# vpc-ccg/circminer

Measured on AMD Instinct MI355X. Metric: paired reads/sec (whole node), hg38 k=20, 2x150 bp; circ_report bit-exact, higher is better.
Workload: dtype int32/u8 (chain scores f64)

## Files before the change

circminer_amd/csrc/cm_core.h:

```cpp
#pragma once
#include <stdint.h>

#include "circminer_hot.h"
#if defined(CM_STAGE2_HOST)
#include <vector>
#endif

#if defined(__HIPCC__)
#define CM_HD __host__ __device__
#define CM_NOINLINE inline
#else
#define CM_HD
#define CM_NOINLINE
#endif

#if !defined(CM_HOOK_DP)
#define CM_HOOK_DP(kind, s, n, t, m) ((void)0)
#endif
#if defined(CM_STATS) && !defined(__HIPCC__)
#if !defined(CM_NSTATS)
#define CM_NSTATS 16
#endif
extern "C" unsigned long long cm_stats[CM_NSTATS];
#define CM_STAT(i, n) ((i) < CM_NSTATS ? (void)(cm_stats[(i) < CM_NSTATS ? (i) : 0] += (unsigned long long)(n)) : (void)0)
// ... 94 lines not shown
constexpr uint32_t MAXUB = 4294967295u;
constexpr int MAXDISCRDTLEN = 20000;
constexpr uint32_t LARIAT2BEGTH = 1000u;
constexpr int DPTINF = 10000000;
constexpr int SC_MAT = 1, SC_MIS = -3, SC_IND = -3, SC_XD = 8;
constexpr int MAX_SEEDS = CM_MAX_CHAIN_FRAGS;
constexpr int MAX_BAND = 8;
constexpr int MAX_TID = 64;
#if defined(CM_STAGE2_HOST)
constexpr int MEMO_N = 512;
#elif defined(CM_MEMO_N)
constexpr int MEMO_N = CM_MEMO_N;
#else
constexpr int MEMO_N = 8;
#endif

enum { ERR_POOL = 1, ERR_SEEDS = 4, ERR_BAND = 8, ERR_MEMO = 16 };

struct KCore {
    cm_params P;
    cm_index_view X;
    AnnotDev A;
    const uint32_t *desc = nullptr;
};
struct Core {
    cm_params P;
    IndexV X;
    AnnotV A;
    g_u32 desc = nullptr;
};
CM_HD inline Core to_core(const KCore &k) {
    Core c;
    c.P = k.P;
    c.X = to_dev(k.X);
    c.A = to_dev(k.A);
    c.desc = (g_u32)k.desc;
    return c;
}

template <class T> CM_HD inline T cmin(T a, T b) { return a < b ? a : b; }
template <class T> CM_HD inline T cmax(T a, T b) { return a > b ? a : b; }
CM_HD inline int cabs(int a) { return a < 0 ? -a : a; }

struct SV {
    g_u8 p;
    int32_t off;
    int32_t step;
    int32_t mode;
    CM_HD inline SV sub(int a) const { return SV{p, off + a * step, step, mode}; }
    CM_HD inline SV rev(int m) const { return SV{p, off + (m - 1) * step, -step, mode}; }
};
struct Read {
    g_u8 p;
    int32_t len;
    int32_t rc;
    CM_HD inline SV view() const { return rc ? SV{p, len - 1, -1, 1} : SV{p, 0, 1, 0}; }
};


// ... 209 lines not shown
        if (e12end < 0 || beg2s2 < 0) continue;
        trans_dist = e12end + beg2s2;
        if (cabs(trans_dist - read_dist) <= c.P.max_ed) return true;
    }
    if (td2intron != -1) {
        trans_dist = td2intron;
        return true;
    }
    trans_dist = INF_I;
    return false;
}

constexpr int SMALL_W = 32;
struct ChainStoreGlobal {
    ChainWork &w;
    g_u32 POS;
    const uint32_t *start;
    const uint32_t *cnt_;
    const uint32_t *base_;
    uint32_t lb_[MAX_SEEDS];
    CM_G Event *ev;
    uint32_t n_ev, cap_ev;
    bool lost;
    CM_HD ChainStoreGlobal(ChainWork &ww, g_u32 pos, const uint32_t *st, const uint32_t *cn, const uint32_t *bs)
        : w(ww), POS(pos), start(st), cnt_(cn), base_(bs), ev(nullptr), n_ev(0), cap_ev(0), lost(false) {}
    CM_HD inline uint32_t cnt(int s) const { return cnt_[s]; }
    CM_HD inline uint32_t base(int s) const { return base_[s]; }
    CM_HD inline uint32_t total(int kc) const { return base_[kc]; }
    CM_HD inline void lb_reset(int kc) { for (int k = 0; k < kc; ++k) lb_[k] = 0; }
    CM_HD inline uint32_t lb(int s) const { return lb_[s]; }
    CM_HD inline void set_lb(int s, uint32_t v) { lb_[s] = v; }
    CM_HD inline void init(uint32_t n_cells, double v) {
        for (uint32_t x = 0; x < n_cells; ++x) {
            w.dp_score[x] = v;
            w.dp_prev[x] = -1;
        }
    }
    CM_HD inline uint32_t pos(int s, uint32_t i) const { return POS[start[s] + i]; }
    CM_HD inline double score(uint32_t x) const { return w.dp_score[x]; }
    CM_HD inline int32_t prev(uint32_t x) const { return w.dp_prev[x]; }
    CM_HD inline void set(uint32_t x, double sc, int32_t pv) {
        w.dp_score[x] = sc;
        w.dp_prev[x] = pv;
    }
    CM_HD inline void push(double sc, uint32_t cell) {
        if (n_ev == cap_ev && !lost) {
            const uint32_t ncap = cap_ev ? cap_ev * 4u : 32u;
            const unsigned long long bytes = (unsigned long long)ncap * sizeof(Event);
            const unsigned long long off = pool_take(w.pool_cursor, bytes);
            if (off + bytes > w.pool_bytes) {
                lost = true;
                flag_err(w.err, ERR_POOL);
            } else {
                CM_G Event *ne = (CM_G Event *)(w.pool + off);
                for (uint32_t q = 0; q < n_ev; ++q) ne[q] = ev[q];
                ev = ne;
                cap_ev = ncap;
            }
        }
        if (n_ev < cap_ev) {
            ev[n_ev].score = sc;
            ev[n_ev].cell = cell;
            ++n_ev;
        }
    }
    CM_HD inline uint32_t n_events() const { return n_ev; }
// ... 1904 lines not shown
```

circminer_amd/csrc/cm_hot.hip:

```cpp
#include <chrono>
#include <hip/hip_runtime.h>
#include <rocprim/device/device_radix_sort.hpp>

#include <algorithm>
#include <atomic>
#include <cstdarg>
#include <cstdio>
#include <cstdlib>
#include <cstring>
#include <string>
#include <functional>
#include <thread>
#include <vector>

#include "circminer_hot.h"
#include "cm_core.h"
#include "cm_aos.h"
#include "cm_index_build.h"

using cmc::Core;
using cmc::KCore;

namespace {

// ... 289 lines not shown
                                                         const int32_t *nchain, const int32_t *high, cm_mapped_read *state, uint8_t *active, int32_t *cat,
                                                         int is_last, int *err, unsigned long long *counters, int str_cap,
                                                         unsigned long long *lane_clk, const uint32_t *perm, const unsigned int *n_light,
                                                         unsigned int *next_chunk, RetryArgs ra) {
    pair_kernel<false>(kc, rd, pair0, n_tile, chains, nchain, high, state, active, cat, is_last, err, counters, str_cap, lane_clk, perm, n_light, next_chunk, ra);
}

template <class T> __device__ inline T wave_excl_scan(T v, int lane, T &total) {
    T x = v;
    for (int o = 1; o < 64; o <<= 1) {
        const T y = __shfl_up(x, o);
        if (lane >= o) x += y;
    }
    total = __shfl(x, 63);
    return x - v;
}
struct HeavyChainCtx {
#if defined(CM_CHAIN_DIAG)
    unsigned long long *tk;
#endif
    const Core *c;
    CM_L const uint32_t *LP;
    CM_L const uint32_t *NB;
    const uint32_t *base, *cnt;
    int kc, seq_len;
    CM_G double *dps;
    CM_G int32_t *dpp;
};
__device__ inline uint32_t heavy_cell(const HeavyChainCtx &h, int ii, uint32_t i, CM_G cmc::Event *ev, double &out_score, int32_t &out_prev,
                                     double &e0, double &e1) {
    const Core &c = *h.c;
    const int kmer = c.P.kmer;
    const uint32_t read_remain = (uint32_t)(h.seq_len - ii * kmer - kmer);
    const int32_t cur_info = (int32_t)h.LP[h.base[ii] + i];
    const uint32_t seg_start = (uint32_t)cur_info, seg_end = (uint32_t)cur_info + kmer - 1;
    uint32_t max_lpos_lim = cmc::MAXUB, max_exon_end = 0;
    int ol = -1;
    double my_score = (double)kmer;
    int32_t my_prev = -1;
    uint32_t n = 0;
    const uint32_t cell = h.base[ii] + i;
    const bool near = (h.NB[cell >> 5] >> (cell & 31)) & 1u;
    uint2 parked = make_uint2(0u, 0u);
    int parked_ol = -1;
    if (near) {
        parked = *(CM_G const uint2 *)(h.dps + cell);
        parked_ol = h.dpp[cell];
    }
#if defined(CM_CHAIN_DIAG)
    if (!ev) h.tk[3] += 1;
#define CD_T0 const unsigned long long cd_t = wall_clock64()
#define CD_ADD(k) h.tk[k] += wall_clock64() - cd_t
#else
#define CD_T0
#define CD_ADD(k)
#endif
    for (int jj = ii + 1; jj < h.kc; ++jj) {
        const uint32_t pcn = h.cnt[jj];
        if (pcn == 0) continue;
        CM_L const uint32_t *pp = h.LP + h.base[jj];
        uint32_t lo = 0, hi = pcn;
        {
            CD_T0;
            while (lo < hi) {
                const uint32_t mid = (lo + hi) >> 1;
                if ((int32_t)pp[mid] <= cur_info) lo = mid + 1;
                else hi = mid;
            }
            CD_ADD(0);
        }
        if (lo >= pcn) continue;
        if (cur_info + c.P.max_intron < (int32_t)pp[lo]) continue;
        if (max_lpos_lim == cmc::MAXUB) {
            CD_T0;
            if (near) {
                max_lpos_lim = parked.x;
                max_exon_end = parked.y;
                ol = parked_ol;
            } else {
                max_exon_end = 0;
                ol = -1;
                max_lpos_lim = seg_start + read_remain + (uint32_t)c.P.max_ed;
            }
            CD_ADD(1);
        }
        const int distr = (jj - ii) * kmer - kmer;
        CD_T0;
        for (uint32_t j = lo; j < pcn && pp[j] <= max_lpos_lim; ++j) {
#if defined(CM_CHAIN_DIAG)
            if (!ev) h.tk[4] += 1;
#endif
            const uint32_t pinfo = pp[j];
            int genome_dist, distt, trans_dist;
            if (max_exon_end == 0 || (pinfo + kmer - 1) <= max_exon_end) genome_dist = (int)(pinfo - seg_end - 1);
            else genome_dist = cmc::INF_I;
            if (cmc::cabs(genome_dist - distr) <= c.P.max_ed) distt = genome_dist;
            else if (cmc::check_junction(c, seg_start, pinfo, ol, kmer, distr, trans_dist)) distt = trans_dist;
            else continue;
            const int maxd = distr < distt ? distt : distr, mind = distr < distt ? distr : distt;
            const double beta = 0.1 * (double)(maxd - mind);
            const double alpha = 2e4 * (double)kmer;
            const double t1 = h.dps[h.base[jj] + j] + alpha;
            const double temp_score = t1 - beta;
            if (temp_score > my_score) {
                my_score = temp_score;
                my_prev = (int32_t)(((uint32_t)jj << 16) | j);
                if (ev) {
                    ev[n].score = temp_score;
                    ev[n].cell = ((uint32_t)ii << 16) | i;
                }
                if (n == 0) e0 = temp_score;
                else if (n == 1) e1 = temp_score;
                ++n;
            }
        }
        CD_ADD(2);
    }
    out_score = my_score;
    out_prev = my_prev;
    return n;
}

struct HeavyBackTrack {
    uint32_t base[cmc::MAX_SEEDS + 1];
    uint32_t cand[CM_BESTCHAINLIM + 2];
// ... 21 lines not shown
    const uint32_t max_best = (uint32_t)c.P.max_chain_len;
    const unsigned int n_heavy = *n_perm;
    auto take = [&]() { return (unsigned int)__shfl((int)(lane == 0 ? atomicAdd(next_problem, 1u) : 0u), 0); };
    for (unsigned int hidx = take(); hidx < n_heavy; hidx = take()) {
        const uint32_t r = perm[hidx];
        const uint64_t p = pair0 + (r >> 2);
        const int mate = (int)((r >> 1) & 1u);
        const int len = (int)(mate ? rd.off2[p + 1] - rd.off2[p] : rd.off1[p + 1] - rd.off1[p]);
#if defined(CM_CHAIN_DIAG)
        const unsigned long long dg0 = wall_clock64();
#endif
        uint32_t st[cmc::MAX_SEEDS], cn[cmc::MAX_SEEDS], base[cmc::MAX_SEEDS + 1];
        int kc = S;
        for (int s = 0; s < S; ++s) {
            st[s] = sstart[(uint64_t)r * S + s];
            cn[s] = scnt[(uint64_t)r * S + s];
        }
        while (kc >= 1 && cn[kc - 1] == 0) --kc;
        base[0] = 0;
        for (int s = 0; s < kc; ++s) base[s + 1] = base[s] + cn[s];
        const uint32_t ncell = base[kc];
        CM_G double *dps = (CM_G double *)(dp_score + celloff[r]);
        CM_G int32_t *dpp = (CM_G int32_t *)(dp_prev + celloff[r]);
        for (int s = 0; s < kc; ++s)
            for (uint32_t i = lane; i < cn[s]; i += 64) LP[base[s] + i] = c.X.pos[st[s] + i];
        for (uint32_t x = lane; x < ncell; x += 64) {
            dps[x] = (double)kmer;
            dpp[x] = -1;
        }
        __threadfence_block();
        __syncthreads();
        CM_L uint32_t *NB = LP + ncell;
        CM_L uint16_t *Q = (CM_L uint16_t *)(NB + 2 * ((ncell + 63) >> 6));
        {
            const uint32_t n_pre = kc >= 1 ? base[kc - 1] : 0u;
            const unsigned long long lt = (1ull << lane) - 1ull;
            uint32_t qn = 0;
            auto look_up = [&](uint32_t cnt) {
                if ((uint32_t)lane < cnt) {
                    const uint32_t x = Q[lane];
                    int ii = 0;
                    for (int s = 1; s < kc; ++s) ii += x >= base[s] ? 1 : 0;
                    const uint32_t read_remain = (uint32_t)(len - ii * kmer - kmer);
                    uint32_t mx = 0;
                    int ol = -1;
                    const uint32_t lim = cmc::upper_bound_lookup(c, LP[x], (uint32_t)kmer, read_remain, mx, ol);
                    *(CM_G uint2 *)(dps + x) = make_uint2(lim, mx);
                    dpp[x] = ol;
                }
            };
            for (uint32_t x0 = 0; x0 < n_pre; x0 += 256) {
                bool nr[4];
#pragma unroll
                for (int u = 0; u < 4; ++u) {
                    const uint32_t x = x0 + 64 * u + lane;
                    nr[u] = x < n_pre && cmc::bit_at(c.A.near_border_bits, c.A.n_bits, LP[x]);
                }
#pragma unroll
                for (int u = 0; u < 4; ++u) {
                    const uint32_t xb = x0 + 64 * u;
                    if (xb >= n_pre) break;
                    const unsigned long long m = __ballot(nr[u]);
                    if (lane == 0) NB[xb >> 5] = (uint32_t)m;
                    if (lane == 32) NB[(xb >> 5) + 1] = (uint32_t)(m >> 32);
                    if (nr[u]) Q[qn + __popcll(m & lt)] = (uint16_t)(xb + lane);
                    qn += (uint32_t)__popcll(m);
                }
                __syncthreads();
                while (qn >= 64) {
                    look_up(64);
                    uint16_t keep[4];
#pragma unroll
                    for (int u = 0; u < 4; ++u) keep[u] = 64u * u + (uint32_t)lane < qn - 64 ? Q[64 + 64 * u + lane] : (uint16_t)0;
                    __syncthreads();
#pragma unroll
                    for (int u = 0; u < 4; ++u)
                        if (64u * u + (uint32_t)lane < qn - 64) Q[64 * u + lane] = keep[u];
                    qn -= 64;
                    __syncthreads();
                }
            }
            if (qn) look_up(qn);
        }
        __threadfence_block();
        __syncthreads();
#if defined(CM_CHAIN_DIAG)
        const unsigned long long dg1 = wall_clock64();
#endif
#if defined(CM_CHAIN_DIAG)
        unsigned long long tk[5] = {0, 0, 0, 0, 0};
        unsigned long long wv[4] = {0, 0, 0, 0};
        HeavyChainCtx H{tk, &c, LP, NB, base, cn, kc, len, dps, dpp};
#else
        HeavyChainCtx H{&c, LP, NB, base, cn, kc, len, dps, dpp};
#endif
        CM_G cmc::Event *ev = nullptr;
        uint32_t n_ev = 0, cap_ev = 0;
        bool lost = false;
        for (int ii = kc - 2; ii >= 0; --ii) {
            for (uint32_t i0 = 0; i0 < cn[ii]; i0 += 64) {
                const uint32_t i = i0 + lane;
                const bool on = i < cn[ii];
                double sc = 0, e0 = 0, e1 = 0;
                int32_t pv = -1;
#if defined(CM_CHAIN_DIAG)
                const unsigned long long w0 = wall_clock64();
#endif
                const uint32_t mine = on ? heavy_cell(H, ii, i, (CM_G cmc::Event *)nullptr, sc, pv, e0, e1) : 0u;
#if defined(CM_CHAIN_DIAG)
                const unsigned long long w1 = wall_clock64();
#endif
                uint32_t total;
                const uint32_t off = wave_excl_scan(mine, lane, total);
                if (n_ev + total > cap_ev && !lost) {
                    uint32_t ncap = cap_ev ? cap_ev : 256u;
                    while (ncap < n_ev + total) ncap *= 4u;
                    const unsigned long long bytes = (unsigned long long)ncap * sizeof(cmc::Event);
                    unsigned long long o = 0;
                    if (lane == 0) o = atomicAdd(pool_cursor, bytes);
                    o = ((unsigned long long)__shfl((unsigned int)(o >> 32), 0) << 32) | (unsigned long long)__shfl((unsigned int)o, 0);
                    if (o + bytes > pool_bytes) {
                        lost = true;
                        if (lane == 0) atomicOr(err, cmc::ERR_POOL);
                    } else {
                        CM_G cmc::Event *ne = (CM_G cmc::Event *)((CM_G uint8_t *)pool + o);
                        for (uint32_t q = lane; q < n_ev; q += 64) ne[q] = ev[q];
                        ev = ne;
                        cap_ev = ncap;
                    }
                }
                if (on) {
                    if (mine && !lost) {
                        CM_G cmc::Event *dst = ev + n_ev + off;
                        if (mine <= 2) {
                            dst[0].score = e0;
                            dst[0].cell = ((uint32_t)ii << 16) | i;
                            if (mine == 2) {
                                dst[1].score = e1;
                                dst[1].cell = ((uint32_t)ii << 16) | i;
                            }
                        } else heavy_cell(H, ii, i, dst, sc, pv, e0, e1);
                    }
                    dps[base[ii] + i] = sc;
                    dpp[base[ii] + i] = pv;
                }
                if (!lost) n_ev += total;
#if defined(CM_CHAIN_DIAG)
                const unsigned long long w3 = wall_clock64();
                wv[0] += w1 - w0;
                wv[2] += w3 - w1;
#endif
            }
#if defined(CM_CHAIN_DIAG)
            const unsigned long long w4 = wall_clock64();
#endif
// ... 50 lines not shown
                        const uint32_t rank = n_c + (uint32_t)__popcll(m & ((1ull << lane) - 1ull));
                        if (hit && rank < max_best) BT.cand[rank] = ev[q].cell;
                        n_c += (uint32_t)__popcll(m);
                        if (n_c > max_best) n_c = max_best;
                    }
                }
                for (int o = 32; o >= 1; o >>= 1) {
                    const double u = __shfl_xor(nxt, o);
                    const int uh = __shfl_xor((int)hv, o);
                    if (uh && (!hv || u > nxt)) {
                        nxt = u;
                        hv = true;
                    }
                }
                __syncthreads();
                if ((uint32_t)lane < n_c) {
                    const uint32_t cell = BT.cand[lane];
                    uint32_t bl = cell >> 16, bi = cell & 0xffffu, n = 0;
                    while (true) {
                        const uint32_t x = BT.base[bl] + bi;
                        BT.cidx[lane][n] = (uint16_t)x;
                        BT.cbl[lane][n] = (uint8_t)bl;
                        ++n;
                        const int32_t pv = dpp[x];
                        if (pv < 0 || n >= (uint32_t)CM_MAX_CHAIN_FRAGS) break;
                        bl = (uint32_t)pv >> 16;
                        bi = (uint32_t)pv & 0xffffu;
                    }
                    BT.clen[lane] = (uint8_t)n;
                }
                __syncthreads();
                const uint32_t first = best_count;
                uint32_t n_emit = 0;
                for (uint32_t a = 0; a < n_c && best_count < max_best; ++a) {
                    if (cur < best_score) {
                        const uint32_t spos = LP[BT.cidx[a][0]];
                        bool mine = false;
                        for (uint32_t x = lane; x < n_rep; x += 64) mine = mine || BT.rep[x] == spos;
                        if (__ballot(mine) != 0ull) continue;
                    }
                    const uint32_t cl = BT.clen[a];
                    if (lane == 0) BT.emit[n_emit] = (uint8_t)a;
                    if ((uint32_t)lane >= 1u && (uint32_t)lane < cl) BT.rep[n_rep + lane - 1] = LP[BT.cidx[a][lane]];
                    if (best_count == 0) {
                        first_q0 = (int)BT.cbl[a][0] * kmer;
                        first_qlast = (int)BT.cbl[a][cl - 1] * kmer;
                    }
// ... 20 lines not shown
                __syncthreads();
                have = hv;
                cur = nxt;
            }
#if defined(CM_CHAIN_DIAG)
            if (lane == 0) {
                atomicAdd(&counters[20], (unsigned long long)n_ev);
                atomicAdd(&counters[21], dg_levels);
                atomicAdd(&counters[22], 1ull);
                atomicAdd(&counters[23], dg_levels * (unsigned long long)((n_ev + 63) / 64));
                atomicAdd(&counters[24], (unsigned long long)ncell);
            }
#endif
        }
        if (best_count == 0) {
            for (int ii = kc - 1; ii >= 0; --ii)
                for (uint32_t i = 0; i < cn[ii]; ++i) {
                    if (best_count >= max_best) break;
                    if (best_count == 0) first_q0 = first_qlast = ii * kmer;
                    if (lane == 0) {
                        CM_G cm_chain &ch = out[best_count];
                        ch.rpos[0] = LP[base[ii] + i];
                        ch.qpos[0] = ii * kmer;
                        ch.score = (float)dps[base[ii] + i];
                        ch.chain_len = 1;
                    }
                    ++best_count;
                }
        }
        __threadfence_block();
        __syncthreads();
        if (lane == 0) {
            nchain[r] = (int32_t)best_count;
            int rs = 0;
            if (best_count > 0) rs = pack_resid(first_q0, len - (first_qlast + kmer));
            resid[r] = (uint16_t)rs;
#if defined(CM_CHAIN_DIAG)
            const unsigned long long dg3 = wall_clock64();
            atomicAdd(&counters[13], dg1 - dg0);
            atomicAdd(&counters[14], dg2 - dg1);
            atomicAdd(&counters[15], dg3 - dg2);
#endif
        }
        __syncthreads();
    }
}

// ... 794 lines not shown
    if (i < n_list) sizes[i] = bucket_off[list[i] + 1] - bucket_off[list[i]];
}
__global__ void __launch_bounds__(BLK) k_ib_over_pack(const uint32_t *bucket_off, const uint32_t *list, const uint32_t *start, uint32_t r0, uint32_t r1,
                                                      const uint16_t *checksum, const uint32_t *pos, uint64_t *keys) {
    const uint32_t base = start[r0];
    for (uint32_t r = r0 + blockIdx.x; r < r1; r += gridDim.x) {
        const uint32_t b0 = bucket_off[list[r]], n = start[r + 1] - start[r], at = start[r] - base;
        for (uint32_t i = threadIdx.x; i < n; i += BLK) keys[at + i] = cmib::over_key(r - r0, checksum[b0 + i], pos[b0 + i]);
    }
}
__global__ void __launch_bounds__(BLK) k_ib_over_unpack(const uint32_t *bucket_off, const uint32_t *list, const uint32_t *start, uint32_t r0, uint32_t r1,
                                                        const uint64_t *keys, uint16_t *checksum, uint32_t *pos) {
    const uint32_t base = start[r0];
    for (uint32_t r = r0 + blockIdx.x; r < r1; r += gridDim.x) {
        const uint32_t b0 = bucket_off[list[r]], n = start[r + 1] - start[r], at = start[r] - base;
        for (uint32_t i = threadIdx.x; i < n; i += BLK) {
            const uint64_t x = keys[at + i];
            checksum[b0 + i] = cmib::key_checksum(x);
            pos[b0 + i] = cmib::key_pos(x);
        }
    }
}

__global__ void k_init_state(KCore kc, cm_mapped_read *state, uint8_t *active, int32_t *cat, uint64_t n) {
    const uint64_t i = (uint64_t)blockIdx.x * BLK + threadIdx.x;
    if (i >= n) return;
    Core c;
    c.P = kc.P;
    cmc::default_mr(c, state[i]);
    active[i] = 1;
    cat[i] = -1;
}

struct Slot {
    bool loaded = false, has_annot = false;
    uint64_t gen = 0;
    uint32_t *d_desc = nullptr;
    bool chain_parallel_ok = false;
    cm_index_view X{};
    cmc::AnnotDev A{};
    std::vector<void *> idx_allocs, ann_allocs;
};

struct ProfRec { hipEvent_t a, b; int cls; };

enum Life { BATCH = 0, CONTEXT = 1 };
struct DevMem {
    void *p = nullptr;
    size_t cap = 0;
    std::vector<DevMem *> *listed = nullptr;
    DevMem() = default;
    DevMem(const DevMem &) = delete;
    DevMem &operator=(const DevMem &) = delete;
};
inline void swap(DevMem &a, DevMem &b) {
    std::swap(a.p, b.p);
    std::swap(a.cap, b.cap);
    if (!a.listed && b.listed) (a.listed = b.listed)->push_back(&a);
    if (!b.listed && a.listed) (b.listed = a.listed)->push_back(&b);
}
template <class T, Life L>
struct DevBuf : DevMem {
    operator T *() const { return (T *)p; }
};
// ... 205 lines not shown
        if (e_ != hipSuccess) return fail(ctx, (e_ == hipErrorOutOfMemory) ? CM_ENOMEM : CM_EHIP, "%s: %s", #call, hipGetErrorString(e_)); \
    } while (0)

void report_hip(cm_ctx *ctx, const char *what, hipError_t e) {
    if (e == hipSuccess) return;
    const int k = ctx ? ctx->teardown_errors++ : 0;
    if (k < 8) fprintf(stderr, "[cmhot] context #%u: %s failed: %s (%d)\n", ctx ? ctx->id : 0u, what, hipGetErrorString(e), (int)e);
}

template <class T>
int up(cm_ctx *ctx, std::vector<void *> &allocs, const T *host, size_t n, const T **dev) {
    void *d = nullptr;
    size_t bytes = (n ? n : 1) * sizeof(T);
    HIPCHK(ctx, hipMalloc(&d, bytes));
    allocs.push_back(d);
    if (n) HIPCHK(ctx, hipMemcpyAsync(d, host, n * sizeof(T), hipMemcpyHostToDevice, ctx->st.B));
    *dev = (const T *)d;
    return CM_OK;
}
void free_all(cm_ctx *ctx, std::vector<void *> &v) {
    for (void *p : v) report_hip(ctx, "hipFree", hipFree(p));
    v.clear();
}
void dfree(cm_ctx *c, DevMem &m) {
    if (m.p) report_hip(c, "hipFree", hipFree(m.p));
    m.p = nullptr;
    m.cap = 0;
}
template <class T, Life L>
hipError_t ensure(cm_ctx *c, DevBuf<T, L> &m, size_t bytes) {
    if (m.p && m.cap >= bytes) return hipSuccess;
    dfree(c, m);
    const hipError_t e = hipMalloc(&m.p, bytes ? bytes : 1);
    if (e != hipSuccess) return e;
    m.cap = bytes;
    if (!m.listed) (m.listed = &c->bufs[L])->push_back(&m);
    return e;
}
void release(cm_ctx *c, Life l) {
    for (DevMem *m : c->bufs[l]) {
        dfree(c, *m);
        m->listed = nullptr;
    }
    c->bufs[l].clear();
}

// ... 25 lines not shown
    hipStream_t st;
    Timer(cm_ctx *ctx, int k, hipStream_t stream = nullptr) : c(ctx), cls(k), on(ctx->prof), st(stream ? stream : ctx->st.B) {
        if (on) {
            r.a = take_event(c);
            r.b = take_event(c);
            r.cls = cls;
            (void)hipEventRecord(r.a, st);
        }
    }
    ~Timer() {
        if (on) {
            (void)hipEventRecord(r.b, st);
            c->recs.push_back(r);
        }
    }
};

KCore make_core(const cm_ctx *c, const Slot &s) {
    KCore k;
    k.P = c->P;
    k.X = s.X;
    k.A = s.A;
    k.desc = s.d_desc;
    return k;
}

int check_slot(cm_ctx *ctx, int slot, bool need_annot) {
    if (slot < 0 || slot >= MAX_SLOTS) return fail(ctx, CM_EINVAL, "slot %d out of range", slot);
    if (!ctx->slots[slot].loaded) return fail(ctx, CM_ESTATE, "contig slot %d not loaded", slot);
    if (need_annot && !ctx->slots[slot].has_annot) return fail(ctx, CM_ESTATE, "annotation of slot %d not loaded", slot);
    return CM_OK;
}

ReadsDev reads_dev(const ReadBufs &r) { return ReadsDev{r.seq1_base + cmc::CM_STAGE_PAD, r.seq2_base + cmc::CM_STAGE_PAD, r.off1, r.off2}; }
ReadsDev current_reads(const cm_ctx *ctx) { return reads_dev(ctx->rd); }

constexpr unsigned HP_PLAN_GRID = 2048;
static bool heavy_pipeline() {
    static const bool v = !(getenv("CM_HEAVY_PIPELINE") && getenv("CM_HEAVY_PIPELINE")[0] == '0');
    return v;
}
static unsigned long long chain_light_w() {
    static const unsigned long long v = getenv("CM_CHAIN_LIGHT_W") ? strtoull(getenv("CM_CHAIN_LIGHT_W"), nullptr, 10) : 256ull;
    return v;
}
static unsigned int chain_light_cells() {
// ... 67 lines not shown
        ctx->seed[s].cls_deferred = false;
    }
    const unsigned long long total = ctx->h_pin[8 + 2 * s];
    const unsigned long long max_cells = ctx->h_pin[9 + 2 * s];
    std::vector<std::pair<uint32_t, uint32_t>> ranges;
    if (total <= ctx->dp.cells_cap) {
        ranges.push_back({0u, n_prob});
    } else {
        ctx->h_celloff.resize((size_t)n_prob + 1);
        HIPCHK(ctx, hipMemcpyAsync(ctx->h_celloff.data(), sb.celloff, ((size_t)n_prob + 1) * sizeof(unsigned long long), hipMemcpyDeviceToHost,
                                   ctx->st.B));
        HIPCHK(ctx, hipStreamSynchronize(ctx->st.B));
        uint32_t a = 0;
        while (a < n_prob) {
            uint32_t b = a;
            while (b < n_prob && ctx->h_celloff[b + 1] - ctx->h_celloff[a] <= ctx->dp.cells_cap) ++b;
            if (b == a) return fail(ctx, CM_ELIMIT, "one chaining problem needs %llu DP cells (> workspace %llu)",
                                    ctx->h_celloff[a + 1] - ctx->h_celloff[a], ctx->dp.cells_cap);
            ranges.push_back({a, b});
            a = b;
        }
    }
    const size_t lds_extra = ((size_t)max_cells / 64 + 2) * 8 + 640;
    const size_t heavy_lds = std::min<size_t>((size_t)S * (size_t)ctx->P.seed_lim * sizeof(uint32_t),
                                              ((size_t)max_cells * sizeof(uint32_t) + 2047) / 2048 * 2048 + 2048) + (lds_extra + 255) / 256 * 256;
    const bool split = ranges.size() == 1 && parallel_ok && heavy_lds <= 152u * 1024u;
    bool fresh = true;
    auto launch_group = [&](uint32_t a, uint32_t b, unsigned long long base, bool use_split) -> int {
        const uint32_t n = b - a;
        if (!fresh) {
            HIPCHK(ctx, hipMemsetAsync(ctx->pool_cursor(s), 0, sizeof(unsigned long long), ctx->st.B));
            HIPCHK(ctx, hipMemsetAsync(sb.cctr + 48, 0, sizeof(unsigned int), ctx->st.B));
        }
        fresh = false;
        if (use_split) {
            HIPCHK(ctx, hipEventRecord(ctx->ev.fork, ctx->st.B));
            HIPCHK(ctx, hipStreamWaitEvent(ctx->st.B2, ctx->ev.fork, 0));
            {
            Timer t(ctx, 6, ctx->st.B2);
            static std::atomic<size_t> heavy_attr{64u * 1024u};
            if (heavy_lds > heavy_attr.load()) {
                HIPCHK(ctx, hipFuncSetAttribute((const void *)k_chain_heavy, hipFuncAttributeMaxDynamicSharedMemorySize, (int)heavy_lds));
                heavy_attr.store(heavy_lds);
            }
            const uint32_t hb = n < 8192u ? n : 8192u;
            hipLaunchKernelGGL(k_chain_heavy, dim3(hb), dim3(64), heavy_lds, ctx->st.B2, core, rd, pair0, S, sb.sstart, sb.scnt, sb.celloff,
                               ctx->dp.score, ctx->dp.prev, ctx->dp.pool, ctx->dp.pool_bytes, ctx->pool_cursor(s), rb.chains, rb.nchain, ctx->d_err,
                               rb.resid, sb.perm4, sb.cctr + CTR_BASE + CHAIN_LIGHT_CLS - 1, sb.cctr + 48, ctx->d_counters);
// ... 138 lines not shown
        if (hwq && !said.exchange(true) && !getenv("CM_QUIET")) fprintf(stderr, "[cmhot] %s\n", ctx->err.c_str());
    }
    *out = ctx;
    return CM_OK;
}

void cm_destroy(cm_ctx *ctx) {
    if (!ctx) return;
    report_hip(ctx, "hipSetDevice", hipSetDevice(ctx->P.device));
    for (const StreamDef &d : STREAMS)
        if (ctx->st.*d.st) report_hip(ctx, (std::string("hipStreamSynchronize(") + d.name + ")").c_str(), hipStreamSynchronize(ctx->st.*d.st));
    report_hip(ctx, "hipGetLastError at teardown", hipGetLastError());
    for (auto e : ctx->ev_free) report_hip(ctx, "hipEventDestroy", hipEventDestroy(e));
    ctx->ev_free.clear();
    for (auto &r : ctx->recs) {
        report_hip(ctx, "hipEventDestroy", hipEventDestroy(r.a));
        report_hip(ctx, "hipEventDestroy", hipEventDestroy(r.b));
    }
    ctx->recs.clear();
    free_reads(ctx);
    for (auto &s : ctx->slots) {
        free_all(ctx, s.idx_allocs);
        free_all(ctx, s.ann_allocs);
    }
    release(ctx, CONTEXT);
    if (ctx->h_pin) report_hip(ctx, "hipHostFree", hipHostFree(ctx->h_pin));
    for (hipEvent_t e : ctx->ev)
        if (e) report_hip(ctx, "hipEventDestroy", hipEventDestroy(e));
    for (const StreamDef &d : STREAMS)
        if (ctx->st.*d.st) report_hip(ctx, "hipStreamDestroy", hipStreamDestroy(ctx->st.*d.st));
    delete ctx;
}

const char *cm_last_error(const cm_ctx *ctx) { return ctx ? ctx->err.c_str() : "null context"; }

static int finish_contig(cm_ctx *ctx, Slot &s) {
    const size_t nb = ((size_t)1 << (2 * CM_WINDOW_SIZE)) + 1;
    s.d_desc = nullptr;
    static const bool use_desc = !(getenv("CM_SEED_DESC") && getenv("CM_SEED_DESC")[0] == '0');
    if (use_desc) {
        const uint64_t n_buckets = nb - 1;
        uint32_t *d = nullptr;
        if (hipMalloc((void **)&d, n_buckets * cmc::DESC_WORDS * sizeof(uint32_t)) == hipSuccess) {
            s.idx_allocs.push_back(d);
            hipLaunchKernelGGL(k_build_desc, dim3((unsigned)((n_buckets + BLK - 1) / BLK)), dim3(BLK), 0, ctx->st.B, s.X.bucket_off, s.X.checksum, n_buckets,
                               ctx->P.kmer, d);
            HIPCHK(ctx, hipGetLastError());
            s.d_desc = d;
        } else (void)hipGetLastError();
    }
    HIPCHK(ctx, hipStreamSynchronize(ctx->st.B));
    s.loaded = true;
    return CM_OK;
}

int cm_load_contig(cm_ctx *ctx, int slot, const cm_index_view *iv) {
    if (!ctx || !iv) return CM_EINVAL;
    if (slot < 0 || slot >= MAX_SLOTS) return fail(ctx, CM_EINVAL, "slot %d out of range", slot);
    if (!iv->genome || !iv->bucket_off || !iv->checksum || !iv->pos) return fail(ctx, CM_EINVAL, "null index array");
    HIPCHK(ctx, hipSetDevice(ctx->P.device));
    Slot &s = ctx->slots[slot];
    free_all(ctx, s.idx_allocs);
    s.d_desc = nullptr;
    s.loaded = false;
    ++s.gen;
    const size_t nb = ((size_t)1 << (2 * CM_WINDOW_SIZE)) + 1;
    s.X = *iv;
    int rc;
    {
        uint8_t *g = nullptr;
        const size_t pad = cmc::CM_STAGE_PAD;
        HIPCHK(ctx, hipMalloc((void **)&g, (size_t)iv->ref_len + 2 * pad));
        s.idx_allocs.push_back(g);
        HIPCHK(ctx, hipMemsetAsync(g, 0, (size_t)iv->ref_len + 2 * pad, ctx->st.B));
        HIPCHK(ctx, hipMemcpyAsync(g + pad, iv->genome, (size_t)iv->ref_len, hipMemcpyHostToDevice, ctx->st.B));
        s.X.genome = g + pad;
    }
    if ((rc = up(ctx, s.idx_allocs, iv->bucket_off, nb, &s.X.bucket_off))) return rc;
    if ((rc = up(ctx, s.idx_allocs, iv->checksum, (size_t)iv->n_entries, &s.X.checksum))) return rc;
    if ((rc = up(ctx, s.idx_allocs, iv->pos, (size_t)iv->n_entries, &s.X.pos))) return rc;
    return finish_contig(ctx, s);
}

static int scan32(cm_ctx *ctx, const uint32_t *in, uint64_t n, uint32_t *out, uint32_t *tmp, uint32_t add, int inclusive) {
    const uint32_t nb = (uint32_t)((n + S32_B - 1) / S32_B);
    if (nb == 0) return CM_OK;
    hipLaunchKernelGGL(k_scan32_a, dim3(nb), dim3(S32_T), 0, ctx->st.B, in, n, out, tmp, add, inclusive);
    hipLaunchKernelGGL(k_scan32_b, dim3(1), dim3(1024), 0, ctx->st.B, tmp, nb);
    hipLaunchKernelGGL(k_scan32_c, dim3(nb), dim3(S32_T), 0, ctx->st.B, out, n, (const uint32_t *)tmp);
    HIPCHK(ctx, hipGetLastError());
    return CM_OK;
}

int cm_load_contig_raw(cm_ctx *ctx, int slot, const cm_index_raw *raw) {
    if (!ctx || !raw) return CM_EINVAL;
    if (slot < 0 || slot >= MAX_SLOTS) return fail(ctx, CM_EINVAL, "slot %d out of range", slot);
    if (!raw->genome || (raw->n_buckets && (!raw->hv || !raw->count14 || !raw->table))) return fail(ctx, CM_EINVAL, "null array in the raw record");
    if (raw->table_slots > 0xffffffffull) return fail(ctx, CM_ELIMIT, "table of %llu slots", (unsigned long long)raw->table_slots);
    HIPCHK(ctx, hipSetDevice(ctx->P.device));
    Slot &s = ctx->slots[slot];
    free_all(ctx, s.idx_allocs);
    s.d_desc = nullptr;
    s.loaded = false;
    ++s.gen;
    const uint64_t n_all = (uint64_t)1 << (2 * CM_WINDOW_SIZE);
    const uint32_t n_b = raw->n_buckets;
    s.X = cm_index_view{};
    s.X.contig_num = raw->contig_num;
    s.X.ref_len = raw->ref_len;
    int rc;
    {
        uint8_t *g = nullptr;
        const size_t pad = cmc::CM_STAGE_PAD;
        HIPCHK(ctx, hipMalloc((void **)&g, (size_t)raw->ref_len + 2 * pad));
        s.idx_allocs.push_back(g);
        HIPCHK(ctx, hipMemsetAsync(g, 0, (size_t)raw->ref_len + 2 * pad, ctx->st.B));
        HIPCHK(ctx, hipMemcpyAsync(g + pad, raw->genome, (size_t)raw->ref_len, hipMemcpyHostToDevice, ctx->st.B));
        s.X.genome = g + pad;
    }
    std::vector<void *> tmp;
    struct FreeTmp {
        cm_ctx *c;
        std::vector<void *> &v;
        ~FreeTmp() { free_all(c, v); }
// ... 176 lines not shown
    s.X.pos = d_ps;
    s.X.n_entries = total;
    if ((rc = finish_contig(ctx, s))) return rc;
    if (stats) {
        float ms = 0.f;
        HIPCHK(ctx, hipEventElapsedTime(&ms, ev_a, ev_b));
        memset(stats, 0, sizeof *stats);
        stats->n_entries = total;
        stats->max_bucket = (uint32_t)st[IB_ST_MAX];
        stats->reserved = (uint32_t)std::min<size_t>(tmp_bytes >> 20, 0xffffffffu);
        for (int i = 0; i < 3; ++i) stats->buckets_by_path[i] = st[IB_ST_PATH + i];
        stats->ms_device = ms;
    }
    return CM_OK;
}

int cm_build_contig(cm_ctx *ctx, int slot, int32_t contig_num, const uint8_t *genome, uint32_t ref_len, cm_build_stats *stats) {
    if (!ctx) return CM_EINVAL;
    if (slot < 0 || slot >= MAX_SLOTS) return fail(ctx, CM_EINVAL, "slot %d out of range", slot);
    if (!genome && ref_len) return fail(ctx, CM_EINVAL, "null genome");
    HIPCHK(ctx, hipSetDevice(ctx->P.device));
    Slot &s = ctx->slots[slot];
    free_all(ctx, s.idx_allocs);
    s.d_desc = nullptr;
    s.loaded = false;
    ++s.gen;
    s.X = cm_index_view{};
    s.X.contig_num = contig_num;
    s.X.ref_len = ref_len;
    hipEvent_t ev_a = take_event(ctx), ev_b = take_event(ctx);
    if (!ev_a || !ev_b) return fail(ctx, CM_EHIP, "hipEventCreate failed");
    const int rc = build_contig_arrays(ctx, s, genome, ref_len, stats, ev_a, ev_b);
    if (rc != CM_OK) {
        (void)hipStreamSynchronize(ctx->st.B);
        (void)hipGetLastError();
        free_all(ctx, s.idx_allocs);
        s.d_desc = nullptr;
        s.loaded = false;
        s.X = cm_index_view{};
    }
    ctx->ev_free.push_back(ev_a);
    ctx->ev_free.push_back(ev_b);
    return rc;
}

int cm_index_download(cm_ctx *ctx, int slot, uint32_t *bucket_off, uint16_t *checksum, uint32_t *pos, uint64_t cap_entries, uint64_t *n_entries) {
// ... 1 lines not shown
    int rc;
    if ((rc = check_slot(ctx, slot, false))) return rc;
    const Slot &s = ctx->slots[slot];
    const uint64_t n = s.X.n_entries;
    if (n_entries) *n_entries = n;
    if (!bucket_off && !checksum && !pos) return CM_OK;
    if ((checksum || pos) && cap_entries < n) return fail(ctx, CM_ELIMIT, "slot %d holds %llu entries, the buffers %llu", slot, (unsigned long long)n, (unsigned long long)cap_entries);
    HIPCHK(ctx, hipSetDevice(ctx->P.device));
    const size_t nb = ((size_t)1 << (2 * CM_WINDOW_SIZE)) + 1;
    if (bucket_off) HIPCHK(ctx, hipMemcpyAsync(bucket_off, s.X.bucket_off, nb * sizeof(uint32_t), hipMemcpyDeviceToHost, ctx->st.B));
    if (checksum && n) HIPCHK(ctx, hipMemcpyAsync(checksum, s.X.checksum, (size_t)n * sizeof(uint16_t), hipMemcpyDeviceToHost, ctx->st.B));
    if (pos && n) HIPCHK(ctx, hipMemcpyAsync(pos, s.X.pos, (size_t)n * sizeof(uint32_t), hipMemcpyDeviceToHost, ctx->st.B));
    HIPCHK(ctx, hipStreamSynchronize(ctx->st.B));
    return CM_OK;
}

int cm_load_annotation(cm_ctx *ctx, int slot, const cm_annot_view *av) {
    if (!ctx || !av) return CM_EINVAL;
    if (slot < 0 || slot >= MAX_SLOTS) return fail(ctx, CM_EINVAL, "slot %d out of range", slot);
    if (av->n_iv == 0 || av->n_chr == 0) return fail(ctx, CM_EINVAL, "annotation needs >= 1 interval and >= 1 chromosome");
    HIPCHK(ctx, hipSetDevice(ctx->P.device));
    Slot &s = ctx->slots[slot];
    free_all(ctx, s.ann_allocs);
    s.has_annot = false;
    ++s.gen;
    cmc::AnnotAosHost aos;
    cmc::build_annot_aos(*av, aos);
    cmc::AnnotDev &A = s.A;
    A = cmc::AnnotDev{};
    A.n_iv = av->n_iv; A.n_seg = av->n_seg; A.n_trans = av->n_trans; A.n_gene = av->n_gene; A.n_chr = av->n_chr; A.n_bits = av->n_bits;
    A.pair_reach = aos.pair_reach;
    int rc;
    auto &al = s.ann_allocs;
    if ((rc = up(ctx, al, aos.iv.data(), aos.iv.size(), &A.iv))) return rc;
    if ((rc = up(ctx, al, av->iv_seg, (size_t)av->iv_seg_off[av->n_iv], &A.iv_seg))) return rc;
    if ((rc = up(ctx, al, aos.seg.data(), aos.seg.size(), &A.seg))) return rc;
    if ((rc = up(ctx, al, av->seg_tid, (size_t)av->seg_tid_off[av->n_seg], &A.seg_tid))) return rc;
    if ((rc = up(ctx, al, aos.tr.data(), aos.tr.size(), &A.tr))) return rc;
    if ((rc = up(ctx, al, av->t2s, (size_t)av->t2s_off[av->n_trans], &A.t2s))) return rc;
    if ((rc = up(ctx, al, aos.gene.data(), aos.gene.size(), &A.gene))) return rc;
    if ((rc = up(ctx, al, av->near_border_bits, (size_t)(av->n_bits / 64), &A.near_border_bits))) return rc;
    if ((rc = up(ctx, al, av->intronic_bits, (size_t)(av->n_bits / 64), &A.intronic_bits))) return rc;
    if ((rc = up(ctx, al, av->chr_shift, (size_t)av->n_chr, &A.chr_shift))) return rc;
    if ((rc = up(ctx, al, av->chr_id, (size_t)av->n_chr, &A.chr_id))) return rc;
    if (av->iv_bucket && av->n_iv_bucket >= 2) {
        if ((rc = up(ctx, al, av->iv_bucket, (size_t)av->n_iv_bucket, &A.iv_bucket))) return rc;
        A.iv_bucket_shift = av->iv_bucket_shift;
        A.n_iv_bucket = av->n_iv_bucket;
    }
    HIPCHK(ctx, hipStreamSynchronize(ctx->st.B));
    {
        const long long mi = ctx->P.max_intron;
        bool ok = mi >= (long long)ctx->P.max_read_len + ctx->P.max_ed && mi < (1ll << 30);
        for (uint32_t i = 0; i < av->n_iv && ok; ++i) {
            if (av->iv_seg_off[i + 1] == av->iv_seg_off[i]) continue;
            const long long far = std::max<long long>((long long)av->iv_max_next_exon[i] + ctx->P.kmer, (long long)av->iv_max_end[i]);
            if (far - (long long)av->iv_spos[i] > mi) ok = false;
        }
        s.chain_parallel_ok = ok;
    }
    s.has_annot = true;
    return CM_OK;
}

int cm_unload_contig(cm_ctx *ctx, int slot) {
    if (!ctx || slot < 0 || slot >= MAX_SLOTS) return CM_EINVAL;
    (void)hipSetDevice(ctx->P.device);
    (void)hipStreamSynchronize(ctx->st.B);
    free_all(ctx, ctx->slots[slot].idx_allocs);
    free_all(ctx, ctx->slots[slot].ann_allocs);
    ctx->slots[slot].loaded = ctx->slots[slot].has_annot = false;
    ctx->slots[slot].d_desc = nullptr;
    ++ctx->slots[slot].gen;
    return CM_OK;
}

static int check_reads(cm_ctx *ctx, const cm_reads *rd, int *max_len_out) {
    const uint64_t n = rd->n_pairs;
    if (n > 0x3fffffffull) return fail(ctx, CM_ELIMIT, "more than 2^30 pairs in one batch");
    if (!rd->seq1 || !rd->seq2 || !rd->off1 || !rd->off2) return fail(ctx, CM_EINVAL, "null read arrays");
    int max_len = 0;
    const uint64_t lim = (uint64_t)ctx->P.max_read_len;
    uint64_t bad = 0, longest = 0;
    auto scan = [&](uint64_t lo, uint64_t hi, uint64_t *bad_o, uint64_t *long_o) {
        uint64_t bd = 0, lg = 0;
        for (uint64_t i = lo; i < hi; ++i) {
            const uint64_t l1 = rd->off1[i + 1] - rd->off1[i], l2 = rd->off2[i + 1] - rd->off2[i];
            const uint64_t m = l1 > l2 ? l1 : l2;
            if (m > lim && !bd) bd = i + 1;
            if (m > lg) lg = m;
        }
        *bad_o = bd;
        *long_o = lg;
// ... 925 lines not shown
```

Before: 28.05 million.

## Track improved DP cells with LDS bitmask and precompute per-entry near-border bits

Drops the global-memory initialisation of the chain DP score/prev arrays. An LDS bitmask now records which cells were actually improved, and reads of cells that were never written fall back to the init value. Near-border bits are precomputed once per index entry at contig/annotation load, so the heavy kernel takes them from a flag packed into the LP high bit instead of doing a random bitmap lookup. The host ChainStoreGlobal gets a similar 128-cell mask. In exchange the kernel does extra bit tests, needs more LDS, and adds a per-load preprocessing kernel plus an extra device buffer.

```diff
diff --git a/circminer_amd/csrc/cm_core.h b/circminer_amd/csrc/cm_core.h
--- a/circminer_amd/csrc/cm_core.h
+++ b/circminer_amd/csrc/cm_core.h
@@ -140,12 +140,14 @@
     cm_index_view X;
     AnnotDev A;
     const uint32_t *desc = nullptr;
+    const uint64_t *entry_near = nullptr;
 };
 struct Core {
     cm_params P;
     IndexV X;
     AnnotV A;
     g_u32 desc = nullptr;
+    g_u64 entry_near = nullptr;
 };
 CM_HD inline Core to_core(const KCore &k) {
     Core c;
@@ -153,6 +155,7 @@
     c.X = to_dev(k.X);
     c.A = to_dev(k.A);
     c.desc = (g_u32)k.desc;
+    c.entry_near = (g_u64)k.entry_near;
     return c;
 }
 
@@ -408,8 +411,13 @@
     CM_G Event *ev;
     uint32_t n_ev, cap_ev;
     bool lost;
+    static constexpr uint32_t MASK_CELLS = 128;
+    uint64_t imp0_, imp1_;
+    bool masked_;
+    double init_;
     CM_HD ChainStoreGlobal(ChainWork &ww, g_u32 pos, const uint32_t *st, const uint32_t *cn, const uint32_t *bs)
-        : w(ww), POS(pos), start(st), cnt_(cn), base_(bs), ev(nullptr), n_ev(0), cap_ev(0), lost(false) {}
+        : w(ww), POS(pos), start(st), cnt_(cn), base_(bs), ev(nullptr), n_ev(0), cap_ev(0), lost(false), imp0_(0), imp1_(0), masked_(false), init_(0) {}
+    CM_HD inline bool stored(uint32_t x) const { return !masked_ || (((x < 64u ? imp0_ : imp1_) >> (x & 63u)) & 1ull); }
     CM_HD inline uint32_t cnt(int s) const { return cnt_[s]; }
     CM_HD inline uint32_t base(int s) const { return base_[s]; }
     CM_HD inline uint32_t total(int kc) const { return base_[kc]; }
@@ -417,17 +425,25 @@
     CM_HD inline uint32_t lb(int s) const { return lb_[s]; }
     CM_HD inline void set_lb(int s, uint32_t v) { lb_[s] = v; }
     CM_HD inline void init(uint32_t n_cells, double v) {
+        masked_ = n_cells <= MASK_CELLS;
+        init_ = v;
+        imp0_ = imp1_ = 0;
+        if (masked_) return;
         for (uint32_t x = 0; x < n_cells; ++x) {
             w.dp_score[x] = v;
             w.dp_prev[x] = -1;
         }
     }
     CM_HD inline uint32_t pos(int s, uint32_t i) const { return POS[start[s] + i]; }
-    CM_HD inline double score(uint32_t x) const { return w.dp_score[x]; }
-    CM_HD inline int32_t prev(uint32_t x) const { return w.dp_prev[x]; }
+    CM_HD inline double score(uint32_t x) const { return stored(x) ? w.dp_score[x] : init_; }
+    CM_HD inline int32_t prev(uint32_t x) const { return stored(x) ? w.dp_prev[x] : -1; }
     CM_HD inline void set(uint32_t x, double sc, int32_t pv) {
         w.dp_score[x] = sc;
         w.dp_prev[x] = pv;
+        if (masked_) {
+            if (x < 64u) imp0_ |= 1ull << x;
+            else imp1_ |= 1ull << (x & 63u);
+        }
     }
     CM_HD inline void push(double sc, uint32_t cell) {
         if (n_ev == cap_ev && !lost) {
diff --git a/circminer_amd/csrc/cm_hot.hip b/circminer_amd/csrc/cm_hot.hip
--- a/circminer_amd/csrc/cm_hot.hip
+++ b/circminer_amd/csrc/cm_hot.hip
@@ -335,11 +335,14 @@
     const Core *c;
     CM_L const uint32_t *LP;
     CM_L const uint32_t *NB;
+    CM_L const uint32_t *IM;
     const uint32_t *base, *cnt;
     int kc, seq_len;
     CM_G double *dps;
     CM_G int32_t *dpp;
 };
+__device__ inline uint32_t heavy_im_word(uint32_t base_s, uint32_t s) { return 2u * ((base_s >> 6) + s); }
+__host__ __device__ inline uint32_t heavy_im_words(uint32_t ncell, uint32_t kc) { return 2u * ((ncell >> 6) + kc + 1u); }
 __device__ inline uint32_t heavy_cell(const HeavyChainCtx &h, int ii, uint32_t i, CM_G cmc::Event *ev, double &out_score, int32_t &out_prev,
                                      double &e0, double &e1) {
     const Core &c = *h.c;
@@ -372,6 +375,7 @@
         const uint32_t pcn = h.cnt[jj];
         if (pcn == 0) continue;
         CM_L const uint32_t *pp = h.LP + h.base[jj];
+        CM_L const uint32_t *im = h.IM + heavy_im_word(h.base[jj], (uint32_t)jj);
         uint32_t lo = 0, hi = pcn;
         {
             CD_T0;
@@ -413,7 +417,8 @@
             const int maxd = distr < distt ? distt : distr, mind = distr < distt ? distr : distt;
             const double beta = 0.1 * (double)(maxd - mind);
             const double alpha = 2e4 * (double)kmer;
-            const double t1 = h.dps[h.base[jj] + j] + alpha;
+            const double prev_score = ((im[j >> 5] >> (j & 31)) & 1u) ? h.dps[h.base[jj] + j] : (double)kmer;
+            const double t1 = prev_score + alpha;
             const double temp_score = t1 - beta;
             if (temp_score > my_score) {
                 my_score = temp_score;
@@ -481,16 +486,20 @@
         const uint32_t ncell = base[kc];
         CM_G double *dps = (CM_G double *)(dp_score + celloff[r]);
         CM_G int32_t *dpp = (CM_G int32_t *)(dp_prev + celloff[r]);
+        CM_L uint32_t *NB = LP + ncell;
+        CM_L uint16_t *Q = (CM_L uint16_t *)(NB + 2 * ((ncell + 63) >> 6));
+        CM_L uint32_t *IM = (CM_L uint32_t *)(Q + 320);
+        const bool by_entry = c.entry_near != nullptr;
         for (int s = 0; s < kc; ++s)
-            for (uint32_t i = lane; i < cn[s]; i += 64) LP[base[s] + i] = c.X.pos[st[s] + i];
-        for (uint32_t x = lane; x < ncell; x += 64) {
-            dps[x] = (double)kmer;
-            dpp[x] = -1;
-        }
+            for (uint32_t i = lane; i < cn[s]; i += 64) {
+                const uint32_t e = st[s] + i;
+                uint32_t v = c.X.pos[e];
+                if (by_entry && s < kc - 1) v |= (uint32_t)((c.entry_near[e >> 6] >> (e & 63)) & 1ull) << 31;
+                LP[base[s] + i] = v;
+            }
+        for (uint32_t x = lane; x < heavy_im_words(ncell, (uint32_t)kc); x += 64) IM[x] = 0u;
         __threadfence_block();
         __syncthreads();
-        CM_L uint32_t *NB = LP + ncell;
-        CM_L uint16_t *Q = (CM_L uint16_t *)(NB + 2 * ((ncell + 63) >> 6));
         {
             const uint32_t n_pre = kc >= 1 ? base[kc - 1] : 0u;
             const unsigned long long lt = (1ull << lane) - 1ull;
@@ -513,7 +522,10 @@
 #pragma unroll
                 for (int u = 0; u < 4; ++u) {
                     const uint32_t x = x0 + 64 * u + lane;
-                    nr[u] = x < n_pre && cmc::bit_at(c.A.near_border_bits, c.A.n_bits, LP[x]);
+                    if (by_entry) {
+                        nr[u] = x < n_pre && (LP[x] >> 31);
+                        if (nr[u]) LP[x] &= 0x7fffffffu;
+                    } else nr[u] = x < n_pre && cmc::bit_at(c.A.near_border_bits, c.A.n_bits, LP[x]);
                 }
 #pragma unroll
                 for (int u = 0; u < 4; ++u) {
@@ -549,9 +561,9 @@
 #if defined(CM_CHAIN_DIAG)
         unsigned long long tk[5] = {0, 0, 0, 0, 0};
         unsigned long long wv[4] = {0, 0, 0, 0};
-        HeavyChainCtx H{tk, &c, LP, NB, base, cn, kc, len, dps, dpp};
+        HeavyChainCtx H{tk, &c, LP, NB, IM, base, cn, kc, len, dps, dpp};
 #else
-        HeavyChainCtx H{&c, LP, NB, base, cn, kc, len, dps, dpp};
+        HeavyChainCtx H{&c, LP, NB, IM, base, cn, kc, len, dps, dpp};
 #endif
         CM_G cmc::Event *ev = nullptr;
         uint32_t n_ev = 0, cap_ev = 0;
@@ -569,6 +581,12 @@
 #if defined(CM_CHAIN_DIAG)
                 const unsigned long long w1 = wall_clock64();
 #endif
+                {
+                    const unsigned long long m = __ballot(mine > 0u);
+                    const uint32_t w = heavy_im_word(base[ii], (uint32_t)ii) + (i0 >> 5);
+                    if (lane == 0) IM[w] = (uint32_t)m;
+                    if (lane == 32) IM[w + 1] = (uint32_t)(m >> 32);
+                }
                 uint32_t total;
                 const uint32_t off = wave_excl_scan(mine, lane, total);
                 if (n_ev + total > cap_ev && !lost) {
@@ -588,8 +606,8 @@
                         cap_ev = ncap;
                     }
                 }
-                if (on) {
-                    if (mine && !lost) {
+                if (on && mine) {
+                    if (!lost) {
                         CM_G cmc::Event *dst = ev + n_ev + off;
                         if (mine <= 2) {
                             dst[0].score = e0;
@@ -686,7 +704,8 @@
                         BT.cidx[lane][n] = (uint16_t)x;
                         BT.cbl[lane][n] = (uint8_t)bl;
                         ++n;
-                        const int32_t pv = dpp[x];
+                        const bool improved = (IM[heavy_im_word(BT.base[bl], bl) + (bi >> 5)] >> (bi & 31)) & 1u;
+                        const int32_t pv = improved ? dpp[x] : -1;
                         if (pv < 0 || n >= (uint32_t)CM_MAX_CHAIN_FRAGS) break;
                         bl = (uint32_t)pv >> 16;
                         bi = (uint32_t)pv & 0xffffu;
@@ -753,7 +772,7 @@
                         CM_G cm_chain &ch = out[best_count];
                         ch.rpos[0] = LP[base[ii] + i];
                         ch.qpos[0] = ii * kmer;
-                        ch.score = (float)dps[base[ii] + i];
+                        ch.score = (float)(double)kmer;
                         ch.chain_len = 1;
                     }
                     ++best_count;
@@ -1594,6 +1613,13 @@
     }
 }
 
+__global__ void __launch_bounds__(BLK) k_entry_near(const uint32_t *pos, uint64_t n_entries, const uint64_t *bits, uint64_t n_bits, uint64_t *out) {
+    const uint64_t e = (uint64_t)blockIdx.x * BLK + threadIdx.x;
+    const bool b = e < n_entries && cmc::bit_at((cmc::g_u64)bits, n_bits, pos[e]);
+    const unsigned long long m = __ballot(b);
+    if ((threadIdx.x & 63) == 0 && e < n_entries) out[e >> 6] = m;
+}
+
 __global__ void k_init_state(KCore kc, cm_mapped_read *state, uint8_t *active, int32_t *cat, uint64_t n) {
     const uint64_t i = (uint64_t)blockIdx.x * BLK + threadIdx.x;
     if (i >= n) return;
@@ -1612,6 +1638,7 @@
     cm_index_view X{};
     cmc::AnnotDev A{};
     std::vector<void *> idx_allocs, ann_allocs;
+    uint64_t *entry_near = nullptr;
 };
 
 struct ProfRec { hipEvent_t a, b; int cls; };
@@ -1863,6 +1890,10 @@
     for (void *p : v) report_hip(ctx, "hipFree", hipFree(p));
     v.clear();
 }
+void drop_entry_near(cm_ctx *ctx, Slot &s) {
+    if (s.entry_near) report_hip(ctx, "hipFree", hipFree(s.entry_near));
+    s.entry_near = nullptr;
+}
 void dfree(cm_ctx *c, DevMem &m) {
     if (m.p) report_hip(c, "hipFree", hipFree(m.p));
     m.p = nullptr;
@@ -1934,6 +1965,7 @@
     k.X = s.X;
     k.A = s.A;
     k.desc = s.d_desc;
+    k.entry_near = s.entry_near;
     return k;
 }
 
@@ -2047,8 +2079,13 @@
         }
     }
     const size_t lds_extra = ((size_t)max_cells / 64 + 2) * 8 + 640;
-    const size_t heavy_lds = std::min<size_t>((size_t)S * (size_t)ctx->P.seed_lim * sizeof(uint32_t),
-                                              ((size_t)max_cells * sizeof(uint32_t) + 2047) / 2048 * 2048 + 2048) + (lds_extra + 255) / 256 * 256;
+    const size_t lds_need = (size_t)max_cells * sizeof(uint32_t) + lds_extra + (size_t)heavy_im_words((uint32_t)max_cells, (uint32_t)S) * sizeof(uint32_t);
+    const size_t heavy_lds = std::max<size_t>(std::min<size_t>((size_t)S * (size_t)ctx->P.seed_lim * sizeof(uint32_t),
+                                                               ((size_t)max_cells * sizeof(uint32_t) + 2047) / 2048 * 2048 + 2048) + (lds_extra + 255) / 256 * 256,
+                                              (lds_need + 255) / 256 * 256);
+#if defined(CM_CHAIN_DIAG)
+    fprintf(stderr, "heavy_lds %zu (largest problem %llu cells)\n", heavy_lds, max_cells);
+#endif
     const bool split = ranges.size() == 1 && parallel_ok && heavy_lds <= 152u * 1024u;
     bool fresh = true;
     auto launch_group = [&](uint32_t a, uint32_t b, unsigned long long base, bool use_split) -> int {
@@ -2233,6 +2270,7 @@
     for (auto &s : ctx->slots) {
         free_all(ctx, s.idx_allocs);
         free_all(ctx, s.ann_allocs);
+        drop_entry_near(ctx, s);
     }
     release(ctx, CONTEXT);
     if (ctx->h_pin) report_hip(ctx, "hipHostFree", hipHostFree(ctx->h_pin));
@@ -2244,6 +2282,25 @@
 }
 
 const char *cm_last_error(const cm_ctx *ctx) { return ctx ? ctx->err.c_str() : "null context"; }
+
+static int make_entry_near(cm_ctx *ctx, Slot &s) {
+    drop_entry_near(ctx, s);
+    if (!s.loaded || !s.has_annot || s.X.n_entries == 0) return CM_OK;
+    if (s.X.ref_len > 0x80000000u) return CM_OK;
+    const uint64_t n = s.X.n_entries;
+    uint64_t *d = nullptr;
+    if (hipMalloc((void **)&d, (size_t)((n + 63) / 64) * sizeof(uint64_t)) != hipSuccess) {
+        (void)hipGetLastError();
+        return CM_OK;
+    }
+    s.entry_near = d;
+    hipLaunchKernelGGL(k_entry_near, dim3((unsigned)((n + BLK - 1) / BLK)), dim3(BLK), 0, ctx->st.B, s.X.pos, n, s.A.near_border_bits, (uint64_t)s.A.n_bits, d);
+    hipError_t e = hipGetLastError();
+    if (e == hipSuccess) e = hipStreamSynchronize(ctx->st.B);
+    if (e != hipSuccess) drop_entry_near(ctx, s);
+    HIPCHK(ctx, e);
+    return CM_OK;
+}
 
 static int finish_contig(cm_ctx *ctx, Slot &s) {
     const size_t nb = ((size_t)1 << (2 * CM_WINDOW_SIZE)) + 1;
@@ -2262,7 +2319,7 @@
     }
     HIPCHK(ctx, hipStreamSynchronize(ctx->st.B));
     s.loaded = true;
-    return CM_OK;
+    return make_entry_near(ctx, s);
 }
 
 int cm_load_contig(cm_ctx *ctx, int slot, const cm_index_view *iv) {
@@ -2272,6 +2329,7 @@
     HIPCHK(ctx, hipSetDevice(ctx->P.device));
     Slot &s = ctx->slots[slot];
     free_all(ctx, s.idx_allocs);
+    drop_entry_near(ctx, s);
     s.d_desc = nullptr;
     s.loaded = false;
     ++s.gen;
@@ -2311,6 +2369,7 @@
     HIPCHK(ctx, hipSetDevice(ctx->P.device));
     Slot &s = ctx->slots[slot];
     free_all(ctx, s.idx_allocs);
+    drop_entry_near(ctx, s);
     s.d_desc = nullptr;
     s.loaded = false;
     ++s.gen;
@@ -2533,6 +2592,7 @@
     HIPCHK(ctx, hipSetDevice(ctx->P.device));
     Slot &s = ctx->slots[slot];
     free_all(ctx, s.idx_allocs);
+    drop_entry_near(ctx, s);
     s.d_desc = nullptr;
     s.loaded = false;
     ++s.gen;
@@ -2580,6 +2640,7 @@
     HIPCHK(ctx, hipSetDevice(ctx->P.device));
     Slot &s = ctx->slots[slot];
     free_all(ctx, s.ann_allocs);
+    drop_entry_near(ctx, s);
     s.has_annot = false;
     ++s.gen;
     cmc::AnnotAosHost aos;
@@ -2618,7 +2679,7 @@
         s.chain_parallel_ok = ok;
     }
     s.has_annot = true;
-    return CM_OK;
+    return make_entry_near(ctx, s);
 }
 
 int cm_unload_contig(cm_ctx *ctx, int slot) {
@@ -2627,6 +2688,7 @@
     (void)hipStreamSynchronize(ctx->st.B);
     free_all(ctx, ctx->slots[slot].idx_allocs);
     free_all(ctx, ctx->slots[slot].ann_allocs);
+    drop_entry_near(ctx, ctx->slots[slot]);
     ctx->slots[slot].loaded = ctx->slots[slot].has_annot = false;
     ctx->slots[slot].d_desc = nullptr;
     ++ctx->slots[slot].gen;
```

After: 28.90 million, median of 6. 3.0% higher.
